# Gongzihang6/Pointcept-KeypointDetection

Measured on AMD Instinct MI355X. Metric: Mpoints/sec PTv3 fwd @100k pts/scene, 1024-pt window; keypoint offset L2 vs ref, higher is better.
Workload: dtype bf16; 1 GPU; OffsetKeypointPTv3 (PT-v3m1 fork config, 46.2M params) eval forward, 1 x 100000-point synthetic surface scene(s) per GPU, patch 1024, serialization + sparse conv + attention + head included; points_per_gpu=100000, parallelism=replicas x1 (scene-sharded, no collective), forwards_in_flight=1

## Files before the change

include/ptv3_hip.h:

```cpp
#ifndef PTV3_HIP_H
#define PTV3_HIP_H
#include <stddef.h>
#include <stdint.h>

#ifdef __cplusplus
extern "C" {
#endif

#define PTV3_F32 0
#define PTV3_BF16 1

#define PTV3_ORDER_Z 0
#define PTV3_ORDER_Z_TRANS 1
#define PTV3_ORDER_HILBERT 2
#define PTV3_ORDER_HILBERT_TRANS 3

#define PTV3_ACT_NONE 0
#define PTV3_ACT_GELU 1
#define PTV3_ACT_RELU 2

const char* ptv3_last_error(void);
int ptv3_version(void);

int ptv3_sfc_encode(const void* grid_coord, int coord_is_i64, const int64_t* batch, int64_t n,
// ... 24 lines not shown
                         void* out, int64_t n, int64_t n_pad, int c, int heads, int patch, float scale,
                         const float* rpe_bias, int dtype, void* stream);

int ptv3_window_attn_varlen_fwd(const void* qkv, const int32_t* win_order, const int32_t* win_inverse,
                                const int32_t* cu_seqlens, int num_windows, void* out, int64_t n, int64_t n_pad,
                                int c, int heads, int max_seqlen, float scale, double sum_len_sq, int dtype,
                                void* stream);

int ptv3_window_attn_rpe_fwd(const void* qkv, const int32_t* win_order, const int32_t* win_inverse, void* out,
                             int64_t n, int64_t n_pad, int c, int heads, int patch, float scale,
                             const int32_t* grid_coord, const float* rpe_table, int pos_bnd, int dtype,
                             void* stream);

int64_t ptv3_subm_table_slots(int64_t n);
int ptv3_subm_build_table(const int32_t* indices, int64_t n, void* table, int64_t slots, void* stream);
int ptv3_subm_neighbors(const int32_t* indices, int64_t n, const void* table, int64_t slots, int ksize,
                        int32_t* nbr, void* stream);

size_t ptv3_subm_block_table_bytes(int64_t n);
int ptv3_subm_build_block_table(const int32_t* indices, int64_t n, void* table, size_t bytes, void* stream);
int ptv3_subm_neighbors_blocks(const int32_t* indices, int64_t n, const void* table, size_t bytes, int ksize,
                               int32_t* nbr, void* stream);

int ptv3_subm_sites(const int64_t* batch, const void* grid_coord, int coord_is_i64, int64_t n, int32_t* indices,
                    int64_t* grid64, void* table, size_t bytes, void* stream);
int ptv3_subm_build_block_table_zeroed(const int32_t* indices, int64_t n, void* table, size_t bytes, void* stream);

size_t ptv3_gemm_workspace_bytes(int64_t m, int cin, int cout, int kvol, int dtype);
int ptv3_gemm_splits(int64_t m, int cin, int cout, int kvol, int dtype);
int ptv3_gemm(const void* x, const void* w, void* out, int64_t m, int cin, int cout, int kvol,
              const int32_t* nbr, const int32_t* row_order, const float* bias, const float* bn_scale,
              const float* bn_shift, int act, const void* res, const int32_t* res_index, void* out2,
              int dtype, void* workspace, size_t workspace_bytes, void* stream);

size_t ptv3_halo_plan_bytes(int64_t m);
int ptv3_halo_plan_shape(int* tile_sites, int* cap_rows);
int ptv3_halo_plan_build(const int32_t* nbr, const int32_t* row_order, int64_t m, void* plan, size_t bytes,
                         void* stream);
int ptv3_conv_halo_policy(int64_t m, int cin, int cout, int kvol, int dtype);
int ptv3_conv_halo(const void* x, const void* w, void* out, int64_t m, int c, const int32_t* nbr,
                   const int32_t* row_order, const void* plan, size_t plan_bytes, const float* bias,
                   const float* bn_scale, const float* bn_shift, int act, const void* res, const int32_t* res_index,
                   void* out2, int dtype, void* stream);
int ptv3_conv_head_halo_policy(int64_t m, int c, int dtype);
int ptv3_conv_head_halo(const void* x, const void* w, const float* conv_bias, int64_t m, int c, const int32_t* nbr,
                        const int32_t* row_order, const void* plan, size_t plan_bytes, const void* shortcut,
                        const float* g0, const float* b0, const float* g1, const float* b1, const void* wqkv,
                        const float* bqkv, void* f1, void* qkv, float eps, int dtype, void* stream);

int ptv3_block_fusable(int c, int hidden, int dtype, int64_t m);
int ptv3_rows_linear_capable(int c, int cout, int dtype, int64_t m);
int ptv3_rows_linear(const void* x, const void* shortcut, const float* g0, const float* b0, const float* g1,
                     const float* b1, const void* w, const float* bias, int act, const void* res, void* f1, void* out,
                     int64_t m, int c, int cout, float eps, int dtype, void* stream);
int ptv3_block_head(const void* x, const float* slab, int splits, const float* conv_bias, const void* shortcut,
                    const float* g0, const float* b0, const float* g1, const float* b1, const void* wqkv,
                    const float* bqkv, void* f1, void* qkv, int64_t m, int c, float eps, int dtype, void* stream);
int ptv3_mlp2_fusable(int cin, int hidden, int cout, int dtype);
int ptv3_mlp2(const void* x, const void* w1, const float* b1, const float* s1, const float* t1, int act,
              const void* w2, const float* b2, void* out, int out_f32, int64_t m, int cin, int hidden, int cout,
              int dtype, void* stream);
int ptv3_block_tail(const void* attn, const void* f1, const void* wproj, const float* bproj, const float* g2,
                    const float* b2, const void* w1, const float* bias1, const void* w2, const float* bias2,
                    void* out, int64_t m, int c, int hidden, float eps, int dtype, void* stream);
int ptv3_block_tail_sliced_policy(int c, int hidden, int dtype, int64_t m);
size_t ptv3_block_tail_sliced_workspace_bytes(int64_t m, int c, int groups);
// ... 392 lines not shown
```

pointcept-keypointdetection_amd/csrc/engine.hip:

```cpp
#include <algorithm>
#include <chrono>
#include <mutex>
#include <stdio.h>
#include <stdlib.h>
#include <vector>
#include "common.h"
#include "window_attn.h"

namespace ptv3 {

struct Arena {
  char* base; size_t cap; size_t off; size_t peak; bool dry; bool failed;
  void* alloc(size_t bytes) {
    size_t a = (off + 255) / 256 * 256;
    off = a + bytes;
    if (off > peak) peak = off;
    if (dry) return (void*)(uintptr_t)256;
    if (off > cap) { failed = true; return nullptr; }
    return base + a;
  }
};

__global__ void make_indices_kernel(const int64_t* __restrict__ batch, const void* __restrict__ grid,
                                    int is_i64, int64_t n, int32_t* __restrict__ idx,
// ... 54 lines not shown
}
static void coord_max(const void* grid, int is_i64, int64_t n, int* state, int* out, const int64_t* offset, int b,
                      int64_t* offset_out, hipStream_t s) {
  const dim3 blocks((unsigned)cdiv(3 * n, 256 * CM_BATCH));
  if (is_i64)
    hipLaunchKernelGGL(coord_max_kernel<int64_t>, blocks, dim3(256), 0, s, (const int64_t*)grid, 3 * n, state, out, offset,
                       b, offset_out);
  else
    hipLaunchKernelGGL(coord_max_kernel<int32_t>, blocks, dim3(256), 0, s, (const int32_t*)grid, 3 * n, state, out, offset,
                       b, offset_out);
}

__global__ void batch_from_offset_kernel(const int64_t* __restrict__ offset, int b, int64_t n,
                                         int64_t* __restrict__ batch) {
  int64_t i = (int64_t)blockIdx.x * blockDim.x + threadIdx.x;
  if (i >= n) return;
  int lo = 0, hi = b;
  while (lo < hi) { int mid = (lo + hi) >> 1; if (offset[mid] > i) hi = mid; else lo = mid + 1; }
  batch[i] = lo;
}

struct Plan {
  int K = -1; int64_t n_pad = 0; int32_t* wo[8] = {nullptr}; int32_t* wi[8] = {nullptr};
  int32_t* cu = nullptr; int nwin = 0; double sum_len_sq = 0.0;
};

struct Level {
  int64_t n = 0; int depth = 0;
  std::vector<int64_t> off_host;
  const int64_t* offset = nullptr;
  const int64_t* grid = nullptr; const int64_t* batch = nullptr;
  int64_t *code = nullptr, *order = nullptr, *inverse = nullptr;
  int32_t* indices = nullptr; void* table = nullptr; size_t table_bytes = 0;
  int32_t* nbr3 = nullptr; int32_t* nbr5 = nullptr; int32_t* row_order = nullptr;
  void* halo = nullptr; size_t halo_bytes = 0; hipEvent_t halo_ready = nullptr; bool halo_waited = false;
  Plan plan[2];
  int32_t* seg = nullptr;
  int64_t* cluster = nullptr;
  int32_t* cluster32 = nullptr;
  hipEvent_t ready = nullptr;
  void* feat = nullptr; void* conv_feat = nullptr; int channels = 0;
};

static inline double now_us() {
  return std::chrono::duration<double, std::micro>(std::chrono::steady_clock::now().time_since_epoch()).count();
}

struct DeviceStreams { hipStream_t geo = nullptr; hipStream_t feat[2] = {nullptr, nullptr}; };
static std::mutex g_pool_mutex;
static std::vector<DeviceStreams> g_device_streams;
static hipStream_t device_stream(int device, int which ) {
  std::lock_guard<std::mutex> guard(g_pool_mutex);
  if ((int)g_device_streams.size() <= device) g_device_streams.resize(device + 1);
  DeviceStreams& d = g_device_streams[device];
  hipStream_t& s = which == 0 ? d.geo : d.feat[which - 1];
  if (!s) {
    if (which == 0) {
      int least = 0, greatest = 0;
      (void)hipDeviceGetStreamPriorityRange(&least, &greatest);
      if (hipStreamCreateWithPriority(&s, hipStreamNonBlocking, greatest) != hipSuccess) s = nullptr;
    } else if (hipStreamCreateWithFlags(&s, hipStreamNonBlocking) != hipSuccess) {
      s = nullptr;
    }
  }
  return s;
}

// ... 147 lines not shown
      int64_t cnt = o - prev;
      n_pad += cnt > K ? (cnt + K - 1) / K * K : cnt;
      prev = o;
    }
    P.K = K; P.n_pad = n_pad;
    bool ragged = false;
    P.nwin = 0; P.sum_len_sq = 0.0; prev = 0;
    for (int64_t o : L.off_host) {
      const int64_t cnt = o - prev;
      prev = o;
      P.nwin += (int)((cnt + K - 1) / K);
      if (cnt < K) { ragged = true; P.sum_len_sq += (double)cnt * cnt; }
      else P.sum_len_sq += (double)((cnt + K - 1) / K) * K * K;
    }
    const int k = d->num_orders;
    int32_t* wo = (int32_t*)G->alloc((size_t)k * n_pad * 4);
    int32_t* wi = (int32_t*)G->alloc((size_t)k * L.n * 4);
    P.cu = (ragged || (dry && d->enable_flash)) ? (int32_t*)G->alloc(((size_t)P.nwin + L.off_host.size() + 1) * 4) : nullptr;
    if (!ragged && !dry) P.cu = nullptr;
    RUN(ptv3_window_plan(L.order, L.inverse, L.offset, (int)L.off_host.size(), k, L.n, n_pad, K, wo, wi, P.cu, sg));
    for (int i = 0; i < k; ++i) { P.wo[i] = wo + (int64_t)i * n_pad; P.wi[i] = wi + (int64_t)i * L.n; }
  }

  hipEvent_t stem_ready = nullptr;
  void level0_sites(Level& L, const void* grid_in, int is_i64) {
    L.indices = (int32_t*)G->alloc((size_t)L.n * 16);
    L.row_order = (int32_t*)G->alloc((size_t)L.n * 4);
    int64_t* g64 = (int64_t*)G->alloc((size_t)L.n * 24);
    L.grid = g64;
    L.table_bytes = ptv3_subm_block_table_bytes(L.n);
    L.table = G->alloc(L.table_bytes);
    RUN(ptv3_subm_sites(L.batch, grid_in, is_i64, L.n, L.indices, g64, L.table, L.table_bytes, sg));
    RUN(ptv3_subm_build_block_table_zeroed(L.indices, L.n, L.table, L.table_bytes, sg));
    L.nbr5 = (int32_t*)G->alloc((size_t)L.n * 125 * 4);
    RUN(ptv3_subm_neighbors_blocks(L.indices, L.n, L.table, L.table_bytes, 5, L.nbr5, sg));
  }

  void level_tables(Level& L, int st) {
    L.nbr3 = (int32_t*)G->alloc((size_t)L.n * 27 * 4);
    RUN(ptv3_subm_neighbors_blocks(L.indices, L.n, L.table, L.table_bytes, 3, L.nbr3, sg));
    const int Ke = patch_K(L, d->enc_patch[st]);
    window_plan(L, L.plan[0], Ke);
    if (!d->enc_mode && st < d->num_stages - 1) {
      const int Kd = patch_K(L, d->dec_patch[st]);
      if (Kd == Ke) L.plan[1] = L.plan[0]; else window_plan(L, L.plan[1], Kd);
    }
  }

  void level_geometry(Level& L, int st, const void* grid_in, int is_i64) {
    L.indices = (int32_t*)G->alloc((size_t)L.n * 16);
    L.row_order = (int32_t*)G->alloc((size_t)L.n * 4);
    if (!dry && ok())
      hipLaunchKernelGGL(make_indices_kernel, dim3((unsigned)cdiv(L.n, 256)), dim3(256), 0, sg, L.batch, grid_in, is_i64,
                         L.n, L.indices, (int64_t*)nullptr, L.row_order, L.order);
    L.table_bytes = ptv3_subm_block_table_bytes(L.n);
    L.table = G->alloc(L.table_bytes);
    RUN(ptv3_subm_build_block_table(L.indices, L.n, L.table, L.table_bytes, sg));
    level_tables(L, st);
  }

  void attention(const Level& L, const Plan& P, const void* qkv, void* out, int C, int H, int oi, float scale) {
    WindowAttnCall a = window_attn_call(qkv, P.wo[oi], P.wi[oi], out, L.n, P.n_pad, C, H, P.K, scale, d->dtype, sf);
    a.cu_seqlens = P.cu; a.num_windows = P.nwin; a.sum_len_sq = P.sum_len_sq;
    RUN(window_attn_forward(a, {"window_attn", WA_RAGGED_OPTIONAL}));
  }

  void block(Level& L, const Plan& P, int C, int H, int oi, bool first = false) {
    const void* conv_w = next(); const float* conv_b = (const float*)next();
// ... 124 lines not shown
  int depth = io->depth;
  const int* hmax = nullptr; const int64_t* hoff = nullptr;
  hipEvent_t read_back = nullptr;
  if (dry) {
    for (int i = 0; i < io->b; ++i) L0.off_host[i] = io->offset_host ? io->offset_host[i] : io->n * (i + 1) / io->b;
    if (depth <= 0) depth = 16;
  } else {
    if (io->offset_host) std::copy(io->offset_host, io->offset_host + io->b, L0.off_host.begin());
    if (depth <= 0 || !io->offset_host) {
      char* pin = (char*)X->pinned_at_least(8 + (size_t)io->b * 8);
      if (!pin) { set_error("forward: cannot allocate the pinned read-back buffer"); return PTV3_ERR_LAUNCH; }
      if (!io->offset_host) hoff = (const int64_t*)(pin + 8);
      if (depth <= 0) {
        int* state = X->coord_max_state();
        if (!state) { set_error("forward: cannot allocate the coordinate-maximum state"); return PTV3_ERR_LAUNCH; }
        hmax = (const int*)pin;
        coord_max(io->grid_coord, io->coord_is_i64, io->n, state, (int*)pin, io->offset, hoff ? io->b : 0,
                  (int64_t*)(pin + 8), sg);
      } else {
        (void)hipMemcpyAsync(pin + 8, io->offset, (size_t)io->b * 8, hipMemcpyDeviceToHost, sg);
      }
      read_back = X->event_at(18);
      (void)hipEventRecord(read_back, sg);
    }
  }
  if (io->batch == nullptr) {
    int64_t* bt = io->batch_out ? io->batch_out : (int64_t*)G.alloc((size_t)io->n * 8);
    if (!dry && R.ok())
      hipLaunchKernelGGL(batch_from_offset_kernel, dim3((unsigned)cdiv(io->n, 256)), dim3(256), 0, sg, io->offset, io->b,
                         io->n, bt);
    L0.batch = bt;
  }
  R.level0_sites(L0, io->grid_coord, io->coord_is_i64);
  if (!dry) {
    if (read_back && X->timed_event_sync(read_back) != hipSuccess) {
      set_error("forward: input read-back failed");
      return PTV3_ERR_LAUNCH;
    }
    if (hoff) std::copy(hoff, hoff + io->b, L0.off_host.begin());
    if (hmax) { depth = 0; for (unsigned v = (unsigned)*hmax + 1; v; v >>= 1) ++depth; }
    PTV3_REQUIRE(depth >= 1 && depth <= 16, "forward: serialization depth %d outside [1,16] (structure.py:81)", depth);
    for (int i = 0; i < io->b; ++i)
      PTV3_REQUIRE(L0.off_host[i] > (i ? L0.off_host[i - 1] : 0), "forward: empty scene %d", i);
    PTV3_REQUIRE(L0.off_host[io->b - 1] == io->n, "forward: offset does not end at n");
  }
  L0.depth = depth;
  if (io->depth_out) *io->depth_out = depth;
  {
    RUNR(ptv3_sfc_encode(io->grid_coord, io->coord_is_i64, L0.batch, io->n, depth, io->order_ids_host, k, L0.code, sg));
    size_t wsb = ptv3_argsort_workspace_bytes(k, io->n);
    void* ws = G.alloc(wsb);
    RUNR(ptv3_argsort_i64_rows(L0.code, k, io->n, std::max(1, 3 * depth + nbits), L0.order, L0.inverse, L0.row_order, ws, wsb,
                               sg));
  }
  if (!dry && R.ok()) { R.stem_ready = X->event_at(19); (void)hipEventRecord(R.stem_ready, sg); }
  R.level_tables(L0, 0);
  if (io->stage_points_host) io->stage_points_host[0] = L0.n;
  if (!dry && R.ok()) { L0.ready = X->event_at(1); (void)hipEventRecord(L0.ready, sg); }
  R.halo_plan(L0, 0);

  auto wait_level = [&](Level& L) { if (!dry && R.ok()) (void)hipStreamWaitEvent(sf, L.ready, 0); };
  struct PoolParams { const void* w; const float *b, *bns, *bnt; };
  const void* stem_w = R.next(); const float* stem_s = (const float*)R.next(); const float* stem_t = (const float*)R.next();
  {
    if (!dry && R.ok()) (void)hipStreamWaitEvent(sf, R.stem_ready, 0);
    const int C0 = d->enc_channels[0];
    L0.feat = F.alloc((size_t)L0.n * C0 * es); L0.channels = C0;
    const void* feat_in = io->feat;
    if (io->raw_feat) {
      void* padded = F.alloc((size_t)L0.n * d->in_channels * es);
      if (!dry && R.ok())
        pad_cast(io->raw_feat, io->raw_feat_dtype, io->raw_feat_channels, padded, d->dtype, d->in_channels, L0.n, sf);
      feat_in = padded;
    }
    R.gemm(feat_in, stem_w, L0.feat, L0.n, d->in_channels, C0, 125, L0.nbr5, L0.row_order, nullptr, stem_s, stem_t,
           PTV3_ACT_GELU, nullptr, nullptr, nullptr);
    L0.conv_feat = L0.feat;
    wait_level(L0);
  }
  for (int st = 0; st < S; ++st) {
    Level& L = lv[st];
    if (st > 0) {
      Level& P = lv[st - 1];
      PoolParams pp;
      pp.w = R.next(); pp.b = (const float*)R.next(); pp.bns = (const float*)R.next(); pp.bnt = (const float*)R.next();
      const int C = d->enc_channels[st], Cp = d->enc_channels[st - 1];
      int pd = 0; { int v = d->stride[st - 1] - 1; while (v > 0) { ++pd; v >>= 1; } }
      if (pd > P.depth) pd = 0;
      P.cluster = (int64_t*)G.alloc((size_t)P.n * 8);
      P.seg = (int32_t*)G.alloc((size_t)(P.n + 1) * 4);
      int64_t* poff = (int64_t*)G.alloc((size_t)io->b * 8);
      int32_t* nout_dev = (int32_t*)G.alloc(256);
      size_t pwsb = ptv3_pool_workspace_bytes(P.n);
      void* pws = G.alloc(pwsb);
      RUNR(ptv3_pool_segments(P.code, P.order, P.n, 3 * pd, P.batch, P.cluster, P.seg, nout_dev, poff, pws, pwsb, sg));
      L.off_host.resize(io->b);
      if (dry) {
        L.off_host = P.off_host;
      } else if (R.ok()) {
        if (hipMemcpyAsync(L.off_host.data(), poff, (size_t)io->b * 8, hipMemcpyDeviceToHost, sg) != hipSuccess ||
            X->timed_sync(sg) != hipSuccess) { set_error("forward: offset read-back failed"); return PTV3_ERR_LAUNCH; }
      }
      if (!R.ok()) break;
      L.n = L.off_host[io->b - 1]; L.depth = P.depth - pd; L.offset = poff; L.channels = C;
      if (io->stage_points_host) io->stage_points_host[st] = L.n;
      const int* perm = io->pool_perm_host + (size_t)(st - 1) * k;
      int64_t* g = (int64_t*)G.alloc((size_t)L.n * 24);
      int64_t* bt = (int64_t*)G.alloc((size_t)L.n * 8);
      L.code = (int64_t*)G.alloc((size_t)k * L.n * 8);
      L.order = (int64_t*)G.alloc((size_t)k * L.n * 8);
      L.inverse = (int64_t*)G.alloc((size_t)k * L.n * 8);
      RUNR(ptv3_pool_reduce(nullptr, nullptr, P.grid, P.batch, P.code, k, P.order, P.seg, P.n, L.n, C, pd, nullptr,
// ... 218 lines not shown
```

pointcept-keypointdetection_amd/ptv3_hip/lib.py:

```python
import ctypes
import os
from ctypes import c_char_p, c_double, c_float, c_int, c_int64, c_size_t, c_uint32, c_void_p

PTV3_F32, PTV3_BF16 = 0, 1
PTV3_PG_TRUNCATED = 16
ACT_NONE, ACT_GELU, ACT_RELU = 0, 1, 2
ORDER_IDS = {"z": 0, "z-trans": 1, "hilbert": 2, "hilbert-trans": 3}

_HERE = os.path.dirname(os.path.abspath(__file__))


def library_path():
    return os.environ.get("PTV3_HIP_LIB", os.path.join(os.path.dirname(_HERE), "lib", "libptv3_hip.so"))


P = c_void_p


class BlockTrain(ctypes.Structure):
    _fields_ = ([("n", c_int64), ("n_pad", c_int64)] +
                [(k, ctypes.c_int32) for k in ("c", "hidden", "heads", "patch", "kvol", "num_windows", "dtype", "reserved")] +
                [("scale", c_float), ("eps", c_float), ("keep1", c_float), ("keep2", c_float), ("sum_len_sq", c_double)] +
                [(k, P) for k in ("nbr", "row_order", "win_order", "win_inverse", "cu_seqlens", "feat", "conv_feat",
                                  "w_conv", "w_lin", "w_qkv", "w_proj", "w_fc1", "w_fc2",
# ... 19 lines not shown
    _fields_ = [(k, P) for k in ("dw1", "db1", "dbn1_weight", "dbn1_bias", "dw2", "db2", "dbn2_weight", "dbn2_bias",
                                 "dw3", "db3")]


SIGNATURES = {
    "ptv3_last_error": (c_char_p, []),
    "ptv3_version": (c_int, []),
    "ptv3_sfc_encode": (c_int, [P, c_int, P, c_int64, c_int, P, c_int, P, P]),
    "ptv3_argsort_workspace_bytes": (c_size_t, [c_int, c_int64]),
    "ptv3_argsort_i64": (c_int, [P, c_int, c_int64, c_int, P, P, P, c_size_t, P]),
    "ptv3_argsort_i64_rows": (c_int, [P, c_int, c_int64, c_int, P, P, P, P, c_size_t, P]),
    "ptv3_argsort_scan_batch": (c_int, []),
    "ptv3_coord_max": (c_int, [P, c_int, c_int64, P, P, P]),
    "ptv3_subm_sites": (c_int, [P, P, c_int, c_int64, P, P, P, c_size_t, P]),
    "ptv3_subm_build_block_table_zeroed": (c_int, [P, c_int64, P, c_size_t, P]),
    "ptv3_pad_plan": (c_int, [P, c_int, c_int64, c_int64, c_int, P, P, P, P]),
    "ptv3_window_maps": (c_int, [P, P, P, P, c_int64, c_int64, P, P, P]),
    "ptv3_window_plan": (c_int, [P, P, P, c_int, c_int, c_int64, c_int64, c_int, P, P, P, P]),
    "ptv3_window_attn_fwd": (c_int, [P, P, P, P, c_int64, c_int64, c_int, c_int, c_int, c_float, P, c_int, P]),
    "ptv3_window_attn_varlen_fwd": (c_int, [P, P, P, P, c_int, P, c_int64, c_int64, c_int, c_int, c_int, c_float,
                                            c_double, c_int, P]),
    "ptv3_window_attn_rpe_fwd": (c_int, [P, P, P, P, c_int64, c_int64, c_int, c_int, c_int, c_float, P, P, c_int,
                                         c_int, P]),
    "ptv3_subm_table_slots": (c_int64, [c_int64]),
    "ptv3_subm_build_table": (c_int, [P, c_int64, P, c_int64, P]),
    "ptv3_subm_neighbors": (c_int, [P, c_int64, P, c_int64, c_int, P, P]),
    "ptv3_subm_block_table_bytes": (c_size_t, [c_int64]),
    "ptv3_subm_build_block_table": (c_int, [P, c_int64, P, c_size_t, P]),
    "ptv3_subm_neighbors_blocks": (c_int, [P, c_int64, P, c_size_t, c_int, P, P]),
    "ptv3_gemm_workspace_bytes": (c_size_t, [c_int64, c_int, c_int, c_int, c_int]),
    "ptv3_gemm": (c_int, [P, P, P, c_int64, c_int, c_int, c_int, P, P, P, P, P, c_int, P, P, P, c_int, P, c_size_t,
                          P]),
    "ptv3_gemm_splits": (c_int, [c_int64, c_int, c_int, c_int, c_int]),
    "ptv3_halo_plan_bytes": (c_size_t, [c_int64]),
    "ptv3_halo_plan_shape": (c_int, [P, P]),
    "ptv3_halo_plan_build": (c_int, [P, P, c_int64, P, c_size_t, P]),
    "ptv3_conv_halo_policy": (c_int, [c_int64, c_int, c_int, c_int, c_int]),
    "ptv3_conv_halo": (c_int, [P, P, P, c_int64, c_int, P, P, P, c_size_t, P, P, P, c_int, P, P, P, c_int, P]),
    "ptv3_block_fusable": (c_int, [c_int, c_int, c_int, c_int64]),
    "ptv3_rows_linear_capable": (c_int, [c_int, c_int, c_int, c_int64]),
    "ptv3_rows_linear": (c_int, [P, P, P, P, P, P, P, P, c_int, P, P, P, c_int64, c_int, c_int, c_float, c_int, P]),
    "ptv3_conv_head_halo_policy": (c_int, [c_int64, c_int, c_int]),
    "ptv3_conv_head_halo": (c_int, [P, P, P, c_int64, c_int, P, P, P, c_size_t, P, P, P, P, P, P, P, P, P, c_float, c_int, P]),
    "ptv3_block_head": (c_int, [P, P, c_int, P, P, P, P, P, P, P, P, P, P, c_int64, c_int, c_float, c_int, P]),
    "ptv3_block_tail": (c_int, [P, P, P, P, P, P, P, P, P, P, P, c_int64, c_int, c_int, c_float, c_int, P]),
    "ptv3_block_tail_sliced_policy": (c_int, [c_int, c_int, c_int, c_int64]),
    "ptv3_block_tail_sliced_workspace_bytes": (c_size_t, [c_int64, c_int, c_int]),
    "ptv3_block_tail_sliced": (c_int, [P, P, P, P, P, P, P, P, P, P, P, c_int64, c_int, c_int, c_float, c_int, c_int, P,
                                       c_size_t, P]),
    "ptv3_rows_linear_ln_capable": (c_int, [c_int, c_int, c_int]),
    "ptv3_rows_linear_ln": (c_int, [P, P, P, P, P, P, c_int64, c_int, c_int, c_float, c_int, c_int, P]),
    "ptv3_subm_conv_ln_capable": (c_int, [c_int, c_int, c_int]),
    "ptv3_subm_conv_ln": (c_int, [P, P, P, P, P, P, P, P, c_int64, c_int, c_int, c_float, c_int, c_int, P]),
    "ptv3_res_conv_capable": (c_int, [c_int64, c_int, c_int, c_int, c_int]),
    "ptv3_res_conv_row_tiles": (c_int, [c_int64, c_int]),
    "ptv3_res_conv": (c_int, [P, P, P, P, P, P, P, P, c_int, P, P, P, P, P, c_int64, c_int, c_int, c_int, c_int, P]),
    "ptv3_mlp2_fusable": (c_int, [c_int, c_int, c_int, c_int]),
    "ptv3_mlp2": (c_int, [P, P, P, P, P, c_int, P, P, P, c_int, c_int64, c_int, c_int, c_int, c_int, P]),
    "ptv3_layernorm": (c_int, [P, P, P, P, P, P, P, P, c_int64, c_int, c_float, c_int, P]),
    "ptv3_layernorm_slabs": (c_int, [P, c_int, P, P, P, P, P, P, P, P, c_int64, c_int, c_float, c_int, P]),
    "ptv3_affine_act": (c_int, [P, P, P, c_int, P, c_int64, c_int, c_int, P]),
    "ptv3_cast": (c_int, [P, c_int, P, c_int, c_int64, P]),
    "ptv3_pool_workspace_bytes": (c_size_t, [c_int64]),
    "ptv3_pool_segments": (c_int, [P, P, c_int64, c_int, P, P, P, P, P, P, c_size_t, P]),
    "ptv3_pool_reduce": (c_int, [P, P, P, P, P, c_int, P, P, c_int64, c_int64, c_int, c_int, P, P, c_int, P, P, P,
                                 P, P, P, c_int, P]),
# ... 155 lines not shown
```

pointcept-keypointdetection_amd/ptv3_hip/ops.py:

```python
import ctypes
from types import SimpleNamespace

import torch

from .lib import lib, PTV3_F32, PTV3_BF16, ACT_NONE, ACT_GELU, ACT_RELU, ORDER_IDS

_DT = {torch.float32: PTV3_F32, torch.bfloat16: PTV3_BF16}

_raw_stream = torch._C._cuda_getCurrentRawStream if hasattr(torch._C, "_cuda_getCurrentRawStream") else None


def _stream():
    if _raw_stream is not None:
        return _raw_stream(torch.cuda.current_device())
    return torch.cuda.current_stream().cuda_stream


def _p(t):
    return None if t is None else t.data_ptr()


def _chk(t, name, dtype=None, dim=None):
    if t is None:
        return
# ... 293 lines not shown
    for t, nm in ((bias, "bias"), (bn_scale, "bn_scale"), (bn_shift, "bn_shift")):
        _chk(t, nm, torch.float32, 1)
    _chk(nbr, "nbr", torch.int32, 2)
    _chk(row_order, "row_order", torch.int32, 1)
    _chk(res, "res", x.dtype, 2)
    _chk(res_index, "res_index", torch.int32, 1)
    cin = x.shape[1]
    cout = w.shape[0]
    if w.numel() != cout * kvol * cin:
        raise RuntimeError(f"gemm: weight has {w.numel()} elements, expected {cout}x{kvol}x{cin}")
    if m is None:
        m = nbr.shape[0] if nbr is not None else x.shape[0]
    if nbr is not None and (nbr.shape[0] != m or nbr.shape[1] != kvol):
        raise RuntimeError("gemm: neighbour table shape mismatch")
    for t in (bias, bn_scale, bn_shift):
        if t is not None and t.numel() != cout:
            raise RuntimeError("gemm: epilogue vector length != cout")
    if res is not None:
        if res.shape[1] != cout or (res_index is None and res.shape[0] != m):
            raise RuntimeError("gemm: residual shape mismatch")
        if res_index is not None and res_index.shape[0] != m:
            raise RuntimeError("gemm: res_index length != m")
    if row_order is not None and row_order.shape[0] != m:
        raise RuntimeError("gemm: row_order length != m")
    out = torch.empty((m, cout), dtype=x.dtype, device=x.device)
    out2 = torch.empty_like(out) if dual else None
    dt = _dt(x)
    ws_bytes = lib.ptv3_gemm_workspace_bytes(m, cin, cout, int(kvol), dt)
    ws = torch.empty(ws_bytes, dtype=torch.uint8, device=x.device) if ws_bytes else None
    lib.check(lib.ptv3_gemm(_p(x), _p(w), _p(out), m, cin, cout, int(kvol), _p(nbr), _p(row_order), _p(bias),
                            _p(bn_scale), _p(bn_shift), int(act), _p(res), _p(res_index), _p(out2), dt, _p(ws),
                            ws_bytes, _stream()), "ptv3_gemm")
    return (out, out2) if dual else out


def halo_plan_shape():
    t, cap = ctypes.c_int(0), ctypes.c_int(0)
    lib.check(lib.ptv3_halo_plan_shape(ctypes.byref(t), ctypes.byref(cap)), "ptv3_halo_plan_shape")
    return t.value, cap.value


def halo_plan(nbr, row_order=None):
    _chk(nbr, "nbr", torch.int32, 2)
    _chk(row_order, "row_order", torch.int32, 1)
    m = nbr.shape[0]
    if nbr.shape[1] != 27:
        raise RuntimeError("halo_plan: the neighbour table must have 27 taps")
    if row_order is not None and row_order.shape[0] != m:
        raise RuntimeError("halo_plan: row_order length != m")
    t, cap = halo_plan_shape()
    tiles = (m + t - 1) // t
    nbytes = lib.ptv3_halo_plan_bytes(m)
    plan = torch.empty(nbytes, dtype=torch.uint8, device=nbr.device)
    lib.check(lib.ptv3_halo_plan_build(_p(nbr), _p(row_order), m, _p(plan), nbytes, _stream()), "ptv3_halo_plan_build")
    cb = (tiles * 4 + 15) // 16 * 16
    rb = tiles * cap * 4
    counts = plan[:tiles * 4].view(torch.int32)
    rows = plan[cb:cb + rb].view(torch.int32).view(tiles, cap)
    slots = plan[cb + rb:cb + rb + tiles * t * 27 * 2].view(torch.int16).view(tiles, t, 27)
    return plan, counts, rows, slots


def conv_halo_policy(m, c, dtype):
    return bool(lib.ptv3_conv_halo_policy(int(m), int(c), int(c), 27, _DT[dtype]))


# ... 1922 lines not shown
```

Baseline: 43.81 Mpoints/s.

## Fuse 5x5x5 neighbour lookup into stem conv and issue it before serialization

```diff
diff --git a/include/ptv3_hip.h b/include/ptv3_hip.h
--- a/include/ptv3_hip.h
+++ b/include/ptv3_hip.h
@@ -80,6 +80,11 @@
               const int32_t* nbr, const int32_t* row_order, const float* bias, const float* bn_scale,
               const float* bn_shift, int act, const void* res, const int32_t* res_index, void* out2,
               int dtype, void* workspace, size_t workspace_bytes, void* stream);
+
+int ptv3_stem_conv_blocks(const void* x, const void* w, void* out, int64_t n, int cin, int cout, int ksize,
+                          const int32_t* indices, const void* table, size_t table_bytes, const int32_t* row_order,
+                          const float* bias, const float* bn_scale, const float* bn_shift, int act, int dtype,
+                          void* stream);
 
 size_t ptv3_halo_plan_bytes(int64_t m);
 int ptv3_halo_plan_shape(int* tile_sites, int* cap_rows);
diff --git a/pointcept-keypointdetection_amd/csrc/block_taps.h b/pointcept-keypointdetection_amd/csrc/block_taps.h
--- /dev/null
+++ b/pointcept-keypointdetection_amd/csrc/block_taps.h
@@ -0,0 +1,49 @@
+#pragma once
+#include "hashtable.h"
+
+namespace ptv3 {
+
+constexpr int BT_NB = 2;
+constexpr int BT_NC = BT_NB * BT_NB * BT_NB;
+
+__device__ __forceinline__ bool bt_candidate(const int4 p, int h, int cc, uint64_t smask, uint64_t& key, uint64_t& slot) {
+  const int cx = cc / (BT_NB * BT_NB), cy = (cc / BT_NB) % BT_NB, cz = cc % BT_NB;
+  const int bx = ((p.y - h) >> 2) + cx, by = ((p.z - h) >> 2) + cy, bz = ((p.w - h) >> 2) + cz;
+  const bool live = bx >= 0 && by >= 0 && bz >= 0 && bx <= ((p.y + h) >> 2) && by <= ((p.z + h) >> 2) &&
+                    bz <= ((p.w + h) >> 2) && bx < 16384 && by < 16384 && bz < 16384;
+  key = block_key(p.x, bx, by, bz);
+  slot = live ? mix64(key) & smask : 0;
+  return live;
+}
+
+__device__ __forceinline__ void bt_probe_on(const BlockSlot* __restrict__ slots, uint64_t smask, uint64_t key, uint64_t slot,
+                                            unsigned long long& m, int32_t& base) {
+  m = 0; base = 0;
+  for (uint64_t probe = 1; probe <= smask; ++probe) {
+    slot = (slot + 1) & smask;
+    const unsigned long long kq = slots[slot].key;
+    if (kq == key) { m = slots[slot].mask; base = slots[slot].base; return; }
+    if (kq == 0) return;
+  }
+}
+
+struct BtLine { unsigned occ; int below[2]; int zr0; };
+__device__ __forceinline__ void bt_line(const int4 p, int h, int dx, int dy, const unsigned long long* __restrict__ cmask,
+                                        const int32_t* __restrict__ cbase, BtLine& ln) {
+  const int x = p.y + dx - h, y = p.z + dy - h;
+  const int cxy = ((((x >> 2) - ((p.y - h) >> 2)) & 1) * BT_NB + (((y >> 2) - ((p.z - h) >> 2)) & 1)) * BT_NB;
+  const int sh = ((x & 3) << 4) | ((y & 3) << 2);
+  const unsigned long long m0 = cmask[cxy], m1 = cmask[cxy + 1];
+  ln.occ = ((unsigned)(m0 >> sh) & 15u) | (((unsigned)(m1 >> sh) & 15u) << 4);
+  ln.below[0] = cbase[cxy] + __popcll(m0 & ((1ull << sh) - 1));
+  ln.below[1] = cbase[cxy + 1] + __popcll(m1 & ((1ull << sh) - 1));
+  ln.zr0 = (p.w - h) & 3;
+}
+__device__ __forceinline__ bool bt_line_tap(const BtLine& ln, int i, int& rank) {
+  const int zr = ln.zr0 + i;
+  const unsigned row = zr < 4 ? ln.occ & 15u : ln.occ >> 4;
+  rank = (zr < 4 ? ln.below[0] : ln.below[1]) + __popc(row & ((1u << (zr & 3)) - 1));
+  return (ln.occ >> zr) & 1;
+}
+
+}
diff --git a/pointcept-keypointdetection_amd/csrc/conv_stem.hip b/pointcept-keypointdetection_amd/csrc/conv_stem.hip
--- /dev/null
+++ b/pointcept-keypointdetection_amd/csrc/conv_stem.hip
@@ -0,0 +1,308 @@
+#include "common.h"
+#include "profile.h"
+#include "halo_tile.h"
+#include "block_taps.h"
+#include "../../include/ptv3_hip.h"
+
+namespace ptv3 {
+
+constexpr int ST_THREADS = 256;
+constexpr int ST_BM = 64;
+constexpr int ST_PD = 2;
+
+struct StemArgs {
+  const int32_t* indices; const BlockSlot* slots; uint64_t smask; const uint32_t* payload;
+  int splits;
+};
+
+template <typename T, int NT, int K, int PD>
+__global__ void __launch_bounds__(ST_THREADS) stem_conv_kernel(GemmArgs a, StemArgs g) {
+  constexpr int BN = 16 * NT;
+  constexpr int KVOL = K * K * K, H = K / 2;
+  typedef Frag<T> F;
+  typedef typename F::type FR;
+  constexpr int E = F::E;
+  constexpr int BK = 2 * F::KC;
+  constexpr int LS = BK + E;
+  constexpr int CPR = BK / E;
+  constexpr int A_LOADS = (ST_BM * CPR) / ST_THREADS;
+  constexpr int B_LOADS = (BN * CPR) / ST_THREADS;
+  constexpr int OS = BN + 16 / (int)sizeof(T);
+  constexpr int SM_OPER = (ST_BM + BN) * LS, SM_OUT = ST_BM * OS;
+  constexpr int SM_ALL = SM_OPER > SM_OUT ? SM_OPER : SM_OUT;
+  constexpr int NCAND = ST_BM * BT_NC;
+  constexpr int CAND_PER = NCAND / ST_THREADS;
+  constexpr int ENT = ST_BM * KVOL;
+  constexpr int LINES = ST_BM * K * K, LIT = (LINES + ST_THREADS - 1) / ST_THREADS;
+  __shared__ __attribute__((aligned(16))) T smem_all[SM_ALL];
+  __shared__ __attribute__((aligned(16))) float sEpi[3 * BN];
+  __shared__ int32_t sNbr[ENT];
+  __shared__ int32_t sRow[ST_BM];
+  static_assert(NCAND * 12 + ST_BM * 16 <= SM_ALL * (int)sizeof(T), "candidate staging overlays the operand tiles");
+  unsigned long long* s_mask = reinterpret_cast<unsigned long long*>(smem_all);
+  int4* s_site = reinterpret_cast<int4*>(s_mask + NCAND);
+  int32_t* s_base = reinterpret_cast<int32_t*>(s_site + ST_BM);
+
+  const T* __restrict__ x = reinterpret_cast<const T*>(a.x);
+  const T* __restrict__ w = reinterpret_cast<const T*>(a.w);
+  const int tid = threadIdx.x, lane = tid & 63, wave = tid >> 6;
+  const int li = lane & 15, g4 = lane >> 4;
+  const int64_t row0 = (int64_t)blockIdx.x * ST_BM;
+  const int n0 = blockIdx.y * BN;
+  const int ktot = KVOL * a.cin;
+  const int nsteps = (ktot + BK - 1) / BK;
+  const int sps = g.splits > 1 ? (nsteps + g.splits - 1) / g.splits : nsteps;
+
+  int a_r[A_LOADS], a_ch[A_LOADS];
+#pragma unroll
+  for (int u = 0; u < A_LOADS; ++u) {
+    const int e = tid * A_LOADS + u;
+    a_r[u] = e / CPR;
+    a_ch[u] = e % CPR;
+  }
+  int b_r[B_LOADS], b_ch[B_LOADS];
+#pragma unroll
+  for (int u = 0; u < B_LOADS; ++u) {
+    const int e = tid * B_LOADS + u;
+    b_r[u] = e / CPR;
+    b_ch[u] = e % CPR;
+  }
+  park_epi(a, sEpi, BN, n0, tid, ST_THREADS);
+
+  {
+    int4 p[CAND_PER];
+    int64_t orow[CAND_PER];
+    bool in[CAND_PER];
+#pragma unroll
+    for (int u = 0; u < CAND_PER; ++u) {
+      const int64_t r = row0 + ((tid + u * ST_THREADS) >> 3);
+      in[u] = r < a.m;
+      orow[u] = in[u] ? (a.row_order ? (int64_t)a.row_order[r] : r) : 0;
+    }
+#pragma unroll
+    for (int u = 0; u < CAND_PER; ++u) p[u] = reinterpret_cast<const int4*>(g.indices)[orow[u]];
+    uint64_t key[CAND_PER], slot[CAND_PER];
+    bool live[CAND_PER];
+    unsigned long long k0[CAND_PER], m0[CAND_PER];
+    int32_t b0[CAND_PER];
+#pragma unroll
+    for (int u = 0; u < CAND_PER; ++u) {
+      live[u] = bt_candidate(p[u], H, (tid + u * ST_THREADS) & 7, g.smask, key[u], slot[u]) && in[u];
+      k0[u] = g.slots[slot[u]].key;
+      m0[u] = g.slots[slot[u]].mask;
+      b0[u] = g.slots[slot[u]].base;
+    }
+#pragma unroll
+    for (int u = 0; u < CAND_PER; ++u) {
+      const int c = tid + u * ST_THREADS;
+      unsigned long long m = 0;
+      int32_t base = 0;
+      if (live[u]) {
+        if (k0[u] == key[u]) { m = m0[u]; base = b0[u]; }
+        else if (k0[u] != 0) bt_probe_on(g.slots, g.smask, key[u], slot[u], m, base);
+      }
+      s_mask[c] = m;
+      s_base[c] = base;
+      if ((c & 7) == 0) { s_site[c >> 3] = p[u]; sRow[c >> 3] = in[u] ? (int32_t)orow[u] : -1; }
+    }
+  }
+  __syncthreads();
+  {
+    uint32_t v[LIT][K];
+    unsigned has[LIT];
+#pragma unroll
+    for (int it = 0; it < LIT; ++it) {
+      const int item = min(tid + it * ST_THREADS, LINES - 1);
+      const int s = item / (K * K), l = item - s * (K * K);
+      BtLine ln;
+      bt_line(s_site[s], H, l / K, l % K, s_mask + s * BT_NC, s_base + s * BT_NC, ln);
+      has[it] = 0;
+#pragma unroll
+      for (int i = 0; i < K; ++i) {
+        int rank;
+        const bool hit = bt_line_tap(ln, i, rank);
+        const int64_t at = hit ? (rank < 0 ? 0 : (rank < a.m ? (int64_t)rank : a.m - 1)) : 0;
+        has[it] |= (unsigned)hit << i;
+        v[it][i] = g.payload[at];
+      }
+    }
+#pragma unroll
+    for (int it = 0; it < LIT; ++it) {
+      const int item = tid + it * ST_THREADS;
+      const int ic = min(item, LINES - 1);
+      const int s = ic / (K * K), l = ic - s * (K * K);
+      const int32_t self = sRow[s];
+#pragma unroll
+      for (int i = 0; i < K; ++i) {
+        int32_t nb = ((has[it] >> i) & 1) ? (int32_t)~v[it][i] : -1;
+        if (l == (K * K) / 2 && i == H) nb = self;
+        if (self < 0) nb = -1;
+        if (item < LINES) sNbr[ic * K + i] = nb;
+      }
+    }
+  }
+  __syncthreads();
+
+  FR rra[PD][A_LOADS], rrb[PD][B_LOADS];
+  unsigned rok[PD];
+  auto issue = [&](int step, FR (&ra)[A_LOADS], FR (&rb)[B_LOADS], unsigned& ok) {
+    const int k0 = step * BK;
+    ok = 0;
+    int64_t src[A_LOADS];
+    int cc[A_LOADS];
+#pragma unroll
+    for (int u = 0; u < A_LOADS; ++u) {
+      const int kk = k0 + E * a_ch[u];
+      const bool in = kk < ktot;
+      const int kks = in ? kk : 0;
+      const int d = a.cin_shift >= 0 ? (kks >> a.cin_shift) : (kks / a.cin);
+      cc[u] = kks - d * a.cin;
+      src[u] = (int64_t)sNbr[a_r[u] * KVOL + d];
+      const bool v = in && src[u] >= 0;
+      ok |= (unsigned)v << u;
+      if (!v) src[u] = 0;
+    }
+#pragma unroll
+    for (int u = 0; u < A_LOADS; ++u) ra[u] = *reinterpret_cast<const FR*>(x + src[u] * a.cin + cc[u]);
+#pragma unroll
+    for (int u = 0; u < B_LOADS; ++u) {
+      const int kk = k0 + E * b_ch[u];
+      const int o = n0 + b_r[u];
+      const bool v = o < a.cout && kk < ktot;
+      ok |= (unsigned)v << (8 + u);
+      rb[u] = *reinterpret_cast<const FR*>(w + (int64_t)(v ? o : 0) * ktot + (v ? kk : 0));
+    }
+  };
+  auto stash = [&](const FR (&ra)[A_LOADS], const FR (&rb)[B_LOADS], unsigned ok) {
+#pragma unroll
+    for (int u = 0; u < A_LOADS; ++u)
+      *reinterpret_cast<FR*>(smem_all + a_r[u] * LS + E * a_ch[u]) = ((ok >> u) & 1u) ? ra[u] : F::zero();
+#pragma unroll
+    for (int u = 0; u < B_LOADS; ++u)
+      *reinterpret_cast<FR*>(smem_all + (ST_BM + b_r[u]) * LS + E * b_ch[u]) = ((ok >> (8 + u)) & 1u) ? rb[u] : F::zero();
+  };
+  const T* sA = smem_all;
+  const T* sB = smem_all + ST_BM * LS;
+
+  f32x4 acc[NT], tot[NT];
+#pragma unroll
+  for (int j = 0; j < NT; ++j) { acc[j] = f32x4{0.f, 0.f, 0.f, 0.f}; tot[j] = f32x4{0.f, 0.f, 0.f, 0.f}; }
+
+#pragma unroll
+  for (int p = 0; p < PD; ++p)
+    if (p < nsteps) issue(p, rra[p], rrb[p], rok[p]);
+  int left = sps;
+  for (int base = 0; base < nsteps; base += PD) {
+#pragma unroll
+    for (int p = 0; p < PD; ++p) {
+      const int step = base + p;
+      if (step >= nsteps) break;
+      stash(rra[p], rrb[p], rok[p]);
+      __syncthreads();
+      if (step + PD < nsteps) issue(step + PD, rra[p], rrb[p], rok[p]);
+#pragma unroll
+      for (int ks = 0; ks < 2; ++ks) {
+        FR xf = *reinterpret_cast<const FR*>(sA + (16 * wave + li) * LS + F::KC * ks + E * g4);
+#pragma unroll
+        for (int j = 0; j < NT; ++j) {
+          FR wf = *reinterpret_cast<const FR*>(sB + (16 * j + li) * LS + F::KC * ks + E * g4);
+          acc[j] = F::mma(wf, xf, acc[j]);
+        }
+      }
+      if (g.splits > 1 && (--left == 0 || step == nsteps - 1)) {
+#pragma unroll
+        for (int j = 0; j < NT; ++j) { tot[j] += acc[j]; acc[j] = f32x4{0.f, 0.f, 0.f, 0.f}; }
+        left = sps;
+      }
+      __syncthreads();
+    }
+  }
+  if (g.splits > 1) {
+#pragma unroll
+    for (int j = 0; j < NT; ++j) acc[j] = tot[j];
+  }
+
+  typedef typename Vec4<T>::type V4;
+  constexpr int N = 16 / (int)sizeof(T);
+  T* out = reinterpret_cast<T*>(a.out);
+  if ((a.cout % N) == 0) {
+#pragma unroll
+    for (int j = 0; j < NT; ++j) {
+      const EpiVec ev = load_epi(sEpi, BN, 16 * j + 4 * g4);
+      float v[4];
+#pragma unroll
+      for (int r = 0; r < 4; ++r) v[r] = epi_value(acc[j][r], ev, r, a.act);
+      *reinterpret_cast<V4*>(smem_all + (size_t)(16 * wave + li) * OS + 16 * j + 4 * g4) = pack4<T>(v[0], v[1], v[2], v[3]);
+    }
+    __syncthreads();
+    constexpr int cpr = BN / N, total = ST_BM * cpr;
+#pragma unroll
+    for (int e = tid; e < total; e += ST_THREADS) {
+      const int rl = e / cpr, col = n0 + (e - rl * cpr) * N;
+      const int32_t orow = sRow[rl];
+      if (orow >= 0 && col < a.cout)
+        *reinterpret_cast<FR*>(out + (int64_t)orow * a.cout + col) = *reinterpret_cast<const FR*>(smem_all + (size_t)rl * OS + (col - n0));
+    }
+    return;
+  }
+  const int32_t orow = sRow[16 * wave + li];
+  if (orow < 0) return;
+#pragma unroll
+  for (int j = 0; j < NT; ++j) {
+    const int ch0 = n0 + 16 * j + 4 * g4;
+    const EpiVec ev = load_epi(sEpi, BN, 16 * j + 4 * g4);
+#pragma unroll
+    for (int r = 0; r < 4; ++r)
+      if (ch0 + r < a.cout) out[(int64_t)orow * a.cout + ch0 + r] = from_f32<T>(epi_value(acc[j][r], ev, r, a.act));
+  }
+}
+
+}
+
+using namespace ptv3;
+
+extern "C" int ptv3_stem_conv_blocks(const void* x, const void* w, void* out, int64_t n, int cin, int cout, int ksize,
+                                     const int32_t* indices, const void* table, size_t table_bytes,
+                                     const int32_t* row_order, const float* bias, const float* bn_scale,
+                                     const float* bn_shift, int act, int dtype, void* stream) {
+  PTV3_REQUIRE(dtype == PTV3_F32 || dtype == PTV3_BF16, "stem_conv_blocks: bad dtype %d", dtype);
+  const int gran = dtype == PTV3_F32 ? 4 : 8;
+  PTV3_REQUIRE(cin > 0 && cin % gran == 0, "stem_conv_blocks: cin=%d must be a positive multiple of %d for this dtype", cin, gran);
+  PTV3_REQUIRE(cout > 0, "stem_conv_blocks: cout=%d", cout);
+  PTV3_REQUIRE(ksize == 3 || ksize == 5, "stem_conv_blocks: ksize %d must be 3 or 5", ksize);
+  PTV3_REQUIRE((bn_scale == nullptr) == (bn_shift == nullptr), "stem_conv_blocks: bn_scale/bn_shift must come together");
+  PTV3_REQUIRE(n >= 0 && n < ((int64_t)1 << 31), "stem_conv_blocks: n=%lld out of range", (long long)n);
+  if (n == 0) return PTV3_OK;
+  PTV3_REQUIRE(x && w && out && indices, "stem_conv_blocks: x, w, out and indices are required");
+  PTV3_REQUIRE(table && table_bytes >= ptv3_subm_block_table_bytes(n) && ((uintptr_t)table & 15) == 0 &&
+                   ((uintptr_t)indices & 15) == 0,
+               "stem_conv_blocks: table must be the one ptv3_subm_build_block_table built for these n sites");
+  const int kvol = ksize * ksize * ksize;
+  int cin_shift = -1;
+  if ((cin & (cin - 1)) == 0) { cin_shift = 0; while ((1 << cin_shift) < cin) ++cin_shift; }
+  GemmArgs a{x, w, out, nullptr, nullptr, nullptr, row_order, nullptr, bias, bn_scale, bn_shift, nullptr,
+             n, cin, cout, kvol, act, cin_shift, 0, 0, 0};
+  const int64_t S = ptv3_subm_table_slots(n);
+  StemArgs g{indices, (const BlockSlot*)table, (uint64_t)(S - 1),
+             (const uint32_t*)((const char*)table + (size_t)S * sizeof(BlockSlot)),
+             ptv3_gemm_splits(n, cin, cout, kvol, dtype)};
+  hipStream_t s = (hipStream_t)stream;
+  const int nt = cout <= 32 ? 2 : 4;
+  const int esz = dtype == PTV3_F32 ? 4 : 2;
+  const int prof = prof_begin(s, PROF_SUBM_CONV, 2.0 * n * kvol * cin * cout,
+                              ((double)n * cin + (double)cout * kvol * cin + (double)n * cout) * esz, nullptr, 0, 0.0);
+  prof_kernel(prof, nt == 2 ? PK_GEMM32_CONV : PK_GEMM64_CONV);
+  const dim3 grid((unsigned)cdiv(n, ST_BM), (unsigned)cdiv(cout, 16 * nt)), block(ST_THREADS);
+#define ST_LAUNCH(T, NT_, K_) hipLaunchKernelGGL((stem_conv_kernel<T, NT_, K_, ST_PD>), grid, block, 0, s, a, g)
+#define ST_PICK(T)                                                        \
+  do {                                                                    \
+    if (ksize == 5) { if (nt == 2) ST_LAUNCH(T, 2, 5); else ST_LAUNCH(T, 4, 5); } \
+    else { if (nt == 2) ST_LAUNCH(T, 2, 3); else ST_LAUNCH(T, 4, 3); }    \
+  } while (0)
+  if (dtype == PTV3_F32) ST_PICK(float); else ST_PICK(__bf16);
+#undef ST_PICK
+#undef ST_LAUNCH
+  prof_end(prof, s);
+  PTV3_LAUNCH_CHECK();
+  return PTV3_OK;
+}
diff --git a/pointcept-keypointdetection_amd/csrc/engine.hip b/pointcept-keypointdetection_amd/csrc/engine.hip
--- a/pointcept-keypointdetection_amd/csrc/engine.hip
+++ b/pointcept-keypointdetection_amd/csrc/engine.hip
@@ -110,7 +110,7 @@
   const int64_t* grid = nullptr; const int64_t* batch = nullptr;
   int64_t *code = nullptr, *order = nullptr, *inverse = nullptr;
   int32_t* indices = nullptr; void* table = nullptr; size_t table_bytes = 0;
-  int32_t* nbr3 = nullptr; int32_t* nbr5 = nullptr; int32_t* row_order = nullptr;
+  int32_t* nbr3 = nullptr; int32_t* row_order = nullptr;
   void* halo = nullptr; size_t halo_bytes = 0; hipEvent_t halo_ready = nullptr; bool halo_waited = false;
   Plan plan[2];
   int32_t* seg = nullptr;
@@ -324,8 +324,7 @@
     L.table = G->alloc(L.table_bytes);
     RUN(ptv3_subm_sites(L.batch, grid_in, is_i64, L.n, L.indices, g64, L.table, L.table_bytes, sg));
     RUN(ptv3_subm_build_block_table_zeroed(L.indices, L.n, L.table, L.table_bytes, sg));
-    L.nbr5 = (int32_t*)G->alloc((size_t)L.n * 125 * 4);
-    RUN(ptv3_subm_neighbors_blocks(L.indices, L.n, L.table, L.table_bytes, 5, L.nbr5, sg));
+    if (!dry && ok()) { stem_ready = X->event_at(19); (void)hipEventRecord(stem_ready, sg); }
   }
 
   void level_tables(Level& L, int st) {
@@ -516,35 +515,6 @@
     L0.batch = bt;
   }
   R.level0_sites(L0, io->grid_coord, io->coord_is_i64);
-  if (!dry) {
-    if (read_back && X->timed_event_sync(read_back) != hipSuccess) {
-      set_error("forward: input read-back failed");
-      return PTV3_ERR_LAUNCH;
-    }
-    if (hoff) std::copy(hoff, hoff + io->b, L0.off_host.begin());
-    if (hmax) { depth = 0; for (unsigned v = (unsigned)*hmax + 1; v; v >>= 1) ++depth; }
-    PTV3_REQUIRE(depth >= 1 && depth <= 16, "forward: serialization depth %d outside [1,16] (structure.py:81)", depth);
-    for (int i = 0; i < io->b; ++i)
-      PTV3_REQUIRE(L0.off_host[i] > (i ? L0.off_host[i - 1] : 0), "forward: empty scene %d", i);
-    PTV3_REQUIRE(L0.off_host[io->b - 1] == io->n, "forward: offset does not end at n");
-  }
-  L0.depth = depth;
-  if (io->depth_out) *io->depth_out = depth;
-  {
-    RUNR(ptv3_sfc_encode(io->grid_coord, io->coord_is_i64, L0.batch, io->n, depth, io->order_ids_host, k, L0.code, sg));
-    size_t wsb = ptv3_argsort_workspace_bytes(k, io->n);
-    void* ws = G.alloc(wsb);
-    RUNR(ptv3_argsort_i64_rows(L0.code, k, io->n, std::max(1, 3 * depth + nbits), L0.order, L0.inverse, L0.row_order, ws, wsb,
-                               sg));
-  }
-  if (!dry && R.ok()) { R.stem_ready = X->event_at(19); (void)hipEventRecord(R.stem_ready, sg); }
-  R.level_tables(L0, 0);
-  if (io->stage_points_host) io->stage_points_host[0] = L0.n;
-  if (!dry && R.ok()) { L0.ready = X->event_at(1); (void)hipEventRecord(L0.ready, sg); }
-  R.halo_plan(L0, 0);
-
-  auto wait_level = [&](Level& L) { if (!dry && R.ok()) (void)hipStreamWaitEvent(sf, L.ready, 0); };
-  struct PoolParams { const void* w; const float *b, *bns, *bnt; };
   const void* stem_w = R.next(); const float* stem_s = (const float*)R.next(); const float* stem_t = (const float*)R.next();
   {
     if (!dry && R.ok()) (void)hipStreamWaitEvent(sf, R.stem_ready, 0);
@@ -557,11 +527,39 @@
         pad_cast(io->raw_feat, io->raw_feat_dtype, io->raw_feat_channels, padded, d->dtype, d->in_channels, L0.n, sf);
       feat_in = padded;
     }
-    R.gemm(feat_in, stem_w, L0.feat, L0.n, d->in_channels, C0, 125, L0.nbr5, L0.row_order, nullptr, stem_s, stem_t,
-           PTV3_ACT_GELU, nullptr, nullptr, nullptr);
+    RUNR(ptv3_stem_conv_blocks(feat_in, stem_w, L0.feat, L0.n, d->in_channels, C0, 5, L0.indices, L0.table, L0.table_bytes,
+                               nullptr, nullptr, stem_s, stem_t, PTV3_ACT_GELU, d->dtype, sf));
     L0.conv_feat = L0.feat;
-    wait_level(L0);
-  }
+  }
+  if (!dry) {
+    if (read_back && X->timed_event_sync(read_back) != hipSuccess) {
+      set_error("forward: input read-back failed");
+      return PTV3_ERR_LAUNCH;
+    }
+    if (hoff) std::copy(hoff, hoff + io->b, L0.off_host.begin());
+    if (hmax) { depth = 0; for (unsigned v = (unsigned)*hmax + 1; v; v >>= 1) ++depth; }
+    PTV3_REQUIRE(depth >= 1 && depth <= 16, "forward: serialization depth %d outside [1,16] (structure.py:81)", depth);
+    for (int i = 0; i < io->b; ++i)
+      PTV3_REQUIRE(L0.off_host[i] > (i ? L0.off_host[i - 1] : 0), "forward: empty scene %d", i);
+    PTV3_REQUIRE(L0.off_host[io->b - 1] == io->n, "forward: offset does not end at n");
+  }
+  L0.depth = depth;
+  if (io->depth_out) *io->depth_out = depth;
+  {
+    RUNR(ptv3_sfc_encode(io->grid_coord, io->coord_is_i64, L0.batch, io->n, depth, io->order_ids_host, k, L0.code, sg));
+    size_t wsb = ptv3_argsort_workspace_bytes(k, io->n);
+    void* ws = G.alloc(wsb);
+    RUNR(ptv3_argsort_i64_rows(L0.code, k, io->n, std::max(1, 3 * depth + nbits), L0.order, L0.inverse, L0.row_order, ws, wsb,
+                               sg));
+  }
+  R.level_tables(L0, 0);
+  if (io->stage_points_host) io->stage_points_host[0] = L0.n;
+  if (!dry && R.ok()) { L0.ready = X->event_at(1); (void)hipEventRecord(L0.ready, sg); }
+  R.halo_plan(L0, 0);
+
+  auto wait_level = [&](Level& L) { if (!dry && R.ok()) (void)hipStreamWaitEvent(sf, L.ready, 0); };
+  struct PoolParams { const void* w; const float *b, *bns, *bnt; };
+  wait_level(L0);
   for (int st = 0; st < S; ++st) {
     Level& L = lv[st];
     if (st > 0) {
diff --git a/pointcept-keypointdetection_amd/ptv3_hip/lib.py b/pointcept-keypointdetection_amd/ptv3_hip/lib.py
--- a/pointcept-keypointdetection_amd/ptv3_hip/lib.py
+++ b/pointcept-keypointdetection_amd/ptv3_hip/lib.py
@@ -75,6 +75,8 @@
     "ptv3_gemm": (c_int, [P, P, P, c_int64, c_int, c_int, c_int, P, P, P, P, P, c_int, P, P, P, c_int, P, c_size_t,
                           P]),
     "ptv3_gemm_splits": (c_int, [c_int64, c_int, c_int, c_int, c_int]),
+    "ptv3_stem_conv_blocks": (c_int, [P, P, P, c_int64, c_int, c_int, c_int, P, P, c_size_t, P, P, P, P, c_int, c_int,
+                                      P]),
     "ptv3_halo_plan_bytes": (c_size_t, [c_int64]),
     "ptv3_halo_plan_shape": (c_int, [P, P]),
     "ptv3_halo_plan_build": (c_int, [P, P, c_int64, P, c_size_t, P]),
diff --git a/pointcept-keypointdetection_amd/ptv3_hip/ops.py b/pointcept-keypointdetection_amd/ptv3_hip/ops.py
--- a/pointcept-keypointdetection_amd/ptv3_hip/ops.py
+++ b/pointcept-keypointdetection_amd/ptv3_hip/ops.py
@@ -349,6 +349,37 @@
                             _p(bn_scale), _p(bn_shift), int(act), _p(res), _p(res_index), _p(out2), dt, _p(ws),
                             ws_bytes, _stream()), "ptv3_gemm")
     return (out, out2) if dual else out
+
+
+def stem_conv_blocks(x, w, indices, table, ksize=5, bias=None, row_order=None, bn_scale=None, bn_shift=None, act=ACT_NONE,
+                     out=None):
+    _chk(x, "x", (torch.float32, torch.bfloat16), 2)
+    _chk(w, "w", x.dtype)
+    for t, nm in ((bias, "bias"), (bn_scale, "bn_scale"), (bn_shift, "bn_shift")):
+        _chk(t, nm, torch.float32, 1)
+    _chk(indices, "indices", torch.int32, 2)
+    _chk(table, "table", torch.uint8, 1)
+    _chk(row_order, "row_order", torch.int32, 1)
+    n, cin = x.shape
+    cout = w.shape[0]
+    if indices.shape[0] != n or indices.shape[1] != 4:
+        raise RuntimeError("stem_conv_blocks: indices must be (n, 4) for the n rows of x")
+    if w.numel() != cout * int(ksize) ** 3 * cin:
+        raise RuntimeError(f"stem_conv_blocks: weight has {w.numel()} elements, expected {cout}x{int(ksize) ** 3}x{cin}")
+    for t in (bias, bn_scale, bn_shift):
+        if t is not None and t.numel() != cout:
+            raise RuntimeError("stem_conv_blocks: epilogue vector length != cout")
+    if row_order is not None and row_order.shape[0] != n:
+        raise RuntimeError("stem_conv_blocks: row_order length != n")
+    if out is None:
+        out = torch.empty((n, cout), dtype=x.dtype, device=x.device)
+    _chk(out, "out", x.dtype, 2)
+    if tuple(out.shape) != (n, cout):
+        raise RuntimeError("stem_conv_blocks: out must be (n, cout)")
+    lib.check(lib.ptv3_stem_conv_blocks(_p(x), _p(w), _p(out), n, cin, cout, int(ksize), _p(indices), _p(table),
+                                        table.numel(), _p(row_order), _p(bias), _p(bn_scale), _p(bn_shift), int(act),
+                                        _dt(x), _stream()), "ptv3_stem_conv_blocks")
+    return out
 
 
 def halo_plan_shape():
```

Result: faster. 44.64 Mpoints/s, median of 6 (+1.9%).
